# Yubo-Shankui/Bind-Your-Avatar-Implementation

Measured on AMD Instinct MI355X. Metric: denoise-steps/sec, higher is better.
Workload: dtype bf16; 1 GPU; BASELINE.json configs[1]: full transformer.forward, 49x480x720 (13x30x45 latent tokens + 226 text), 2 characters (2 ID + 2 audio), batch 1, random-init 8.6B-param architecture; layers=42, batch=1, launch=eager, parallelism=single GPU

## Files before the change

bind_your_avatar_implementation_amd/_hip.py:

```python
import ctypes
import os

from .build import LIB_PATH as _BUILT_LIB

LIB_PATH = os.environ.get("BYA_HIP_LIB") or _BUILT_LIB

_c = ctypes
_vp, _i32, _i64, _f32 = _c.c_void_p, _c.c_int32, _c.c_int64, _c.c_float


class GemmDesc(_c.Structure):
    _fields_ = [("M", _i32), ("N", _i32), ("K", _i32), ("batch", _i32),
                ("lda", _i32), ("ldw", _i32), ("ldc", _i32), ("ldres", _i32),
                ("a_batch_stride", _i64), ("c_batch_stride", _i64), ("res_batch_stride", _i64),
                ("gate_batch_stride", _i64), ("gate_split", _i32), ("act", _i32),
                ("n_split", _i32), ("c_split_stride", _i64), ("bias_rowscale", _vp), ("alpha", _f32)]


class GemmPlan(_c.Structure):
    _fields_ = [("path", _i32), ("m0", _i32), ("tail", _i32), ("split_k", _i32), ("row_chunks", _i32)]


class QkNormDesc(_c.Structure):
    _fields_ = [("qw", _vp), ("qb", _vp), ("kw", _vp), ("kb", _vp), ("cos", _vp), ("sin", _vp),
# ... 91 lines not shown

class SchedCoef(_c.Structure):
    _fields_ = [("guidance", _f32), ("sqrt_alpha", _f32), ("sqrt_beta", _f32), ("k_sample", _f32),
                ("k_denoised", _f32), ("k_noise", _f32), ("k_cur", _f32), ("k_old", _f32)]


SIGNATURES = {
    "bya_abi_version": [],
    "bya_set_option": [_i32, _i32],
    "bya_get_option": [_i32, _c.POINTER(_i32)],
    "bya_mfma_calibration": [_vp, _i64, _vp, _i32, _vp],
    "bya_gemm_bf16": [_vp, _vp, _vp, _vp, _vp, _vp, _vp, _c.POINTER(GemmDesc), _vp],
    "bya_gemm_skinny_bf16": [_vp, _vp, _vp, _vp, _vp, _c.POINTER(GemmDesc), _vp],
    "bya_gemm_qkv_norm_rope": [_vp, _vp, _vp, _vp, _c.POINTER(GemmDesc), _c.POINTER(QkNormDesc), _vp],
    "bya_gemm_bf16_plan": [_vp, _vp, _vp, _vp, _vp, _vp, _vp, _c.POINTER(GemmDesc), _c.POINTER(GemmPlan)],
    "bya_gemm_qkv_norm_rope_plan": [_vp, _vp, _vp, _vp, _c.POINTER(GemmDesc), _c.POINTER(QkNormDesc), _c.POINTER(GemmPlan)],
    "bya_gemm_qkv_norm_rope_stats": [_vp, _vp, _vp, _vp, _c.POINTER(GemmDesc), _c.POINTER(QkNormDesc), _vp, _i32, _vp],
    "bya_gemm_qkv_norm_rope_stats_plan": [_vp, _vp, _vp, _vp, _c.POINTER(GemmDesc), _c.POINTER(QkNormDesc), _vp, _i32, _c.POINTER(GemmPlan)],
    "bya_set_gemm_workspace": [_vp, _i64],
    "bya_gemm_workspace_bytes": [_c.POINTER(_i64)],
    "bya_gemm_workspace_status": [_c.POINTER(_i32), _vp],
    "bya_quantize_rows_fp8": [_vp, _vp, _vp, _i32, _i32, _i64, _i64, _vp],
    "bya_gemm_fp8": [_vp, _vp, _vp, _vp, _vp, _vp, _vp, _vp, _vp, _c.POINTER(GemmDesc), _vp],
    "bya_gemm_fp8_plan": [_vp, _vp, _vp, _vp, _vp, _vp, _vp, _vp, _vp, _c.POINTER(GemmDesc), _c.POINTER(GemmPlan)],
    "bya_gemm_fp8_qkv_norm_rope": [_vp, _vp, _vp, _vp, _vp, _vp, _c.POINTER(GemmDesc), _c.POINTER(QkNormDesc), _vp],
    "bya_gemm_fp8_qkv_norm_rope_plan": [_vp, _vp, _vp, _vp, _vp, _vp, _c.POINTER(GemmDesc), _c.POINTER(QkNormDesc),
                                        _c.POINTER(GemmPlan)],
    "bya_gemm_fp8_qkv_norm_rope_stats": [_vp, _vp, _vp, _vp, _vp, _vp, _c.POINTER(GemmDesc), _c.POINTER(QkNormDesc), _vp, _i32, _vp],
    "bya_gemm_fp8_qkv_norm_rope_stats_plan": [_vp, _vp, _vp, _vp, _vp, _vp, _c.POINTER(GemmDesc), _c.POINTER(QkNormDesc), _vp, _i32,
                                              _c.POINTER(GemmPlan)],
# ... 101 lines not shown
    "bya_p2p_push_verified": [_vp, _i32, _i64, _vp, _i32, _i32, _vp, _vp, _vp, _vp, _vp, _vp],
    "bya_p2p_exchange_verified": [_vp, _i32, _i64, _vp, _i32, _i32, _vp, _vp, _i64, _vp, _vp, _vp, _vp, _vp],
    "bya_p2p_verify": [_vp, _vp, _vp, _i32, _i32, _vp, _vp, _vp],
    "bya_p2p_poison": [_vp, _i32, _vp, _i64, _vp],
    "bya_p2p_alloc": [_i64, _i32, _c.POINTER(_vp)],
    "bya_p2p_free": [_vp],
    "bya_p2p_ipc_export": [_vp, _vp],
    "bya_p2p_ipc_import": [_vp, _c.POINTER(_vp)],
    "bya_p2p_ipc_release": [_vp],
    "bya_cfg_scheduler_step": [_vp, _i32, _i64, _vp, _vp, _vp, _vp, _vp, _i64, _c.POINTER(SchedCoef), _vp],
    "bya_cfg_scheduler_step_plan": [_vp, _i32, _i64, _vp, _vp, _i64, _c.POINTER(SchedCoef), _c.POINTER(StepPlan)],
}

OPTIONS = {"gemm_splitk": 0, "gemm_splitk_min": 1, "gemm_tile": 2, "gemm_variant": 3, "attn_streamk": 4, "fp8_kernel": 5,
           "p2p_groups": 6, "reference_forms": 7, "mx_kernel": 8}
REFERENCE_FORMS = {"rowgemm_chunked": 1, "kv_mix_generic": 2, "ln_generic": 4, "router_scores_wave": 8, "attn_narrow_store": 16}
def _named_value(var, v, table):
    if v not in table:
        raise ValueError(f"{var}={v!r}: expected one of {sorted(table)}")
    return table[v]


ENV_OPTIONS = {
    "BYA_GEMM_SPLITK": ("gemm_splitk", int),
    "BYA_GEMM_SPLITK_MIN": ("gemm_splitk_min", int),
    "BYA_GEMM_TILE": ("gemm_tile", int),
    "BYA_GEMM_VARIANT": ("gemm_variant", lambda v: {"w8": 1, "no128": 2}.get(v, 0)),
    "BYA_ATTN_STREAMK": ("attn_streamk", int),
    "BYA_FP8_KERNEL": ("fp8_kernel", lambda v: 1 if v.startswith("1") else 0),
    "BYA_P2P_GROUPS": ("p2p_groups", int),
    "BYA_MX_KERNEL": ("mx_kernel", lambda v: _named_value("BYA_MX_KERNEL", v, {"0": 0, "1": 1, "p256": 1, "2": 2, "always": 2})),
# ... 69 lines not shown
```

bind_your_avatar_implementation_amd/csrc/gemm.hip:

```cpp
#include "gemm_common.h"
#include <stdlib.h>
#include <string.h>
#include "options.h"

namespace {


template <int ROWS, int NWAVES>
__device__ __forceinline__ void stage_tile(const bf16_t* __restrict__ src, int ld, int row0, int row_max, int k0,
                                           char* lds_tile, int wave, int lane) {
    constexpr int PER_WAVE = ROWS / NWAVES;
#pragma unroll
    for (int q = 0; q < PER_WAVE / 8; ++q) {
        const int rbase = wave * PER_WAVE + q * 8;
        const int rl = rbase + (lane >> 3);
        const int chunk = (lane & 7) ^ ((rl >> 1) & 7);
        int gr = row0 + rl;
        gr = gr < row_max ? gr : row_max;
        const bf16_t* g = src + (long long)gr * ld + k0 + chunk * 8;
        __builtin_amdgcn_global_load_lds(GLOBAL_PTR(g), LDS_PTR(lds_tile + rbase * 128), 16, 0, 0);
    }
}

__device__ __forceinline__ bf16x8 lds_frag(const char* tile, int row, int chunk) {
// ... 211 lines not shown
            load_frag_b<0>(bx, cW0);
            if (t + 2 < nk) { piece(t + 2, 0); piece(t + 2, 1); }
        }
        __builtin_amdgcn_sched_barrier(0);
        mfma_quadrant<1, 0>(acc, a1, by);
        __builtin_amdgcn_sched_barrier(0);
    }
    asm volatile("s_waitcnt lgkmcnt(0)" ::: "memory");

    auto run = [&](auto act_tag) {
        epilogue_block<decltype(act_tag)::value, 4, 8, 2>(p, z, m0 + wm * 128 + fr, n0 + wn * 64 + fq * 4, acc);
    };
    dispatch_act_big(p.act, run);
}

inline bool v4_eligible(const GemmArgs& a) {
    return a.K >= 3 * BK && a.N % 8 == 0 && a.n_split % 8 == 0 && a.ldc % 8 == 0 && (!a.res || a.ldres % 8 == 0) &&
        !(((uintptr_t)a.C | (uintptr_t)a.res | (uintptr_t)a.bias | (uintptr_t)a.gate0 | (uintptr_t)a.gate1) & 15) &&
        a.c_bs % 8 == 0 && a.res_bs % 8 == 0 && a.gate_bs % 8 == 0 && a.c_split_stride % 8 == 0;
}

inline bool p128_eligible(const GemmArgs& a) { return v4_eligible(a) && a.K >= 4 * BK && a.conv_cpg_log2 < 0 && bya_opt(BYA_OPT_GEMM_VARIANT) == 0; }

inline int path256(const GemmArgs& a) {
    return v4_eligible(a) && bya_opt(BYA_OPT_GEMM_VARIANT) != 1 ? BYA_GEMM_PATH_P256 : BYA_GEMM_PATH_W8_256;
}

int launch_w8_256(const GemmArgs& a, int batch, hipStream_t s) {
    const int tiles_m = (a.M + 255) / 256, tiles_n = (a.N + 255) / 256;
    dim3 grid(tiles_m * tiles_n, 1, batch);
    const size_t lds = 2 * 512 * BK * 2;
    static std::atomic<unsigned long long> attr_done{0};
    if (bya_allow_big_lds(reinterpret_cast<const void*>(gemm256_kernel), (int)lds, attr_done) != BYA_OK) return BYA_ERR_LAUNCH;
    BYA_LAUNCH(gemm256_kernel, grid, dim3(512), lds, s, a);
    return hipGetLastError() == hipSuccess ? BYA_OK : BYA_ERR_LAUNCH;
}

// ... 2 lines not shown
    const int tiles_m = (a.M + BM - 1) / BM, tiles_n = (a.N + BN - 1) / BN;
    dim3 grid(tiles_m * tiles_n, 1, batch);
    const size_t lds = 2 * (BM + BN) * BK * 2;
    static std::atomic<unsigned long long> attr_done{0};
    if (bya_allow_big_lds(reinterpret_cast<const void*>(gemm_bf16_kernel<BM, BN, WAVES_M, WAVES_N>), (int)lds, attr_done) != BYA_OK)
        return BYA_ERR_LAUNCH;
    BYA_LAUNCH((gemm_bf16_kernel<BM, BN, WAVES_M, WAVES_N>), grid, dim3(64 * WAVES_M * WAVES_N), lds, s, a);
    return hipGetLastError() == hipSuccess ? BYA_OK : BYA_ERR_LAUNCH;
}

constexpr double REL_128S = 0.85, REL_128P = 0.80;
inline double rounds_128(int M, int N, int batch, double rel) {
    const long long t = (long long)((M + 127) / 128) * ((N + 255) / 256) * batch;
    return 0.5 * (double)((t + 255) / 256) / rel;
}
inline double rounds_256_split(int M, int N, int K, int batch) {
    const long long tiles = (long long)((M + 255) / 256) * ((N + 255) / 256) * batch, full = tiles / 256, rem = tiles % 256;
    if (rem == 0) return (double)full;
    const int R = (int)((rem + 7) / 8);
    int parts = 32 / R;
    const int by_k = (K / BK) / bya_gemm_split_min_ktiles();
    if (parts > by_k) parts = by_k;
    return (double)full + (parts > 1 ? 1.0 / parts + 0.3 : 1.0);
}
inline int hybrid_rows(int M, int N, int batch, double rel, double* cost) {
    const long long tn = (N + 255) / 256, tiles = (long long)((M + 255) / 256) * tn, full = tiles / 256;
    if (batch != 1 || full < 1 || tiles % 256 == 0) return 0;
    const int main_tm = (int)(full * 256 / tn), m0 = main_tm * 256;
    if (m0 <= 0 || m0 >= M) return 0;
    *cost = (double)(((long long)main_tm * tn + 255) / 256) + rounds_128(M - m0, N, 1, rel) + 0.05;
    return m0;
}
inline int plan_rows_qkn(int M, int N, int batch, int* m0) {
    const int forced = bya_opt(BYA_OPT_GEMM_TILE);
    if (forced >= 0) return forced == 5 || forced == 6 ? 1 : 0;
    const long long t256 = (long long)((M + 255) / 256) * ((N + 255) / 256) * batch;
    const double r256 = (double)((t256 + 255) / 256), r128 = rounds_128(M, N, batch, REL_128P);
    double best = r256, hc = 0.0;
    int plan = 0;
    if (r128 < 0.97 * best) { best = r128; plan = 1; }
    const int hm = hybrid_rows(M, N, batch, REL_128P, &hc);
    if (hm > 0 && hc < (plan == 0 ? r256 - 0.15 : 0.97 * best)) { *m0 = hm; plan = 2; }
    return plan;
}

// ... 9 lines not shown
    const double t256x128 = rounds(256, 128, 1) / 0.95;
    const double frac_rounds = (double)((M + 255) / 256) * ((N + 255) / 256) * batch / 256.0;
    const double t256 = splitk ? (frac_rounds + 0.12) * 65536.0 : rounds(256, 256, 1) / 1.00;
    (void)t256x128;
#ifdef BYA_GEMM_NO_DEEP_GRID
    const bool deep_grid = false;
#else
    const bool deep_grid = frac_rounds >= 4.0 && M >= 512 && K >= 512;
#endif
    if (((M < 1024 || K < 1024) && !deep_grid) || N < 512 || !act_on_big_tiles(act)) return 1;
    if (p128_ok) {
        const double t256s = (splitk ? rounds_256_split(M, N, K, batch) * 65536.0 : t256) / 1.2;
        const double best = t256s <= t128 ? t256s : t128, r128 = rounds_128(M, N, batch, REL_128S);
        if (r128 * 65536.0 / 1.2 < 0.97 * best) {
            double hc = 0.0;
            if (!splitk && hybrid_rows(M, N, batch, REL_128S, &hc) > 0 && hc < 0.97 * r128 && t256 / 1.2 <= t128) return 4;
            return 6;
        }
    }
    return (t256 / 1.2 <= t128) ? 4 : 1;
}

}

namespace {
constexpr int MAX_DEVICES = 64;
std::atomic<void*> g_gemm_ws[MAX_DEVICES];
inline int current_device() {
    int dev = 0;
    return hipGetDevice(&dev) == hipSuccess && dev >= 0 && dev < MAX_DEVICES ? dev : -1;
}
// ... 15 lines not shown
    if (!ws) return BYA_OK;
    unsigned word = 0;
    if (hipMemcpyAsync(&word, ws + 1023 * 4, 4, hipMemcpyDeviceToHost, stream) != hipSuccess) return BYA_ERR_LAUNCH;
    if (hipStreamSynchronize(stream) != hipSuccess) return BYA_ERR_LAUNCH;
    *timeouts = (int32_t)word;
    return BYA_OK;
}

extern "C" int bya_gemm_workspace_bytes(int64_t* bytes) {
    if (!bytes) return BYA_ERR_SHAPE;
    *bytes = (int64_t)GEMM_WS_BYTES;
    return BYA_OK;
}

namespace {
int dispatch_gemm(const GemmArgs& a, int nbatch, hipStream_t stream, bya_gemm_plan* plan);

int bf16_args(const void* A, const void* W, const void* bias, const void* C, const void* res, const void* gate0,
              const void* gate1, const bya_gemm_desc* d, GemmArgs* out) {
    if (!A || !W || !C || !d) return BYA_ERR_SHAPE;
    if (d->M <= 0 || d->N <= 0 || d->K <= 0 || d->batch <= 0) return BYA_ERR_SHAPE;
    if (d->K % BK != 0 || d->N % 4 != 0) return BYA_ERR_SHAPE;
    if (d->lda % 8 || d->ldw % 8) return BYA_ERR_ALIGN;
    if (((uintptr_t)A | (uintptr_t)W) & 15) return BYA_ERR_ALIGN;
    const int rc = gemm_epilogue_check(C, res, bias, gate0, gate1, d, d->act >= 0 && d->act <= 6);
    if (rc != BYA_OK) return rc;
    gemm_fill_args(A, W, bias, C, res, gate0, gate1, d, out);
    const int dev = current_device();
    char* const ws = dev < 0 ? nullptr : static_cast<char*>(g_gemm_ws[dev].load());
    out->ws_counters = reinterpret_cast<unsigned*>(ws);
    out->ws_slabs = ws ? reinterpret_cast<float*>(ws + GEMM_WS_COUNTER_BYTES) : nullptr;
// ... 9 lines not shown
    if (rcs != BYA_OK) return rcs;
    if (d->M <= 0 || d->N <= 0 || d->K <= 0 || d->batch <= 0 || d->K % BK != 0) return BYA_ERR_SHAPE;
    if ((d->N != 3 * n->width && d->N != 2 * n->width) || n->width % 128 != 0 || d->n_split <= 0 || d->act != 0 || d->bias_rowscale || (d->alpha != 0.0f && d->alpha != 1.0f))
        return BYA_ERR_UNSUPPORTED;
    if (d->lda % 8 || d->ldw % 8) return BYA_ERR_ALIGN;
    if (((uintptr_t)A | (uintptr_t)W | (uintptr_t)C | (uintptr_t)bias | (uintptr_t)n->qw | (uintptr_t)n->qb | (uintptr_t)n->kw |
         (uintptr_t)n->kb | (uintptr_t)n->cos | (uintptr_t)n->sin) & 15) return BYA_ERR_ALIGN;
    gemm_fill_args(A, W, bias, C, nullptr, nullptr, nullptr, d, out);
    out->ldres = 0; out->res_bs = 0; out->gate_bs = 0; out->gate_split = 0;
    qkn_fill_norm(n, out);
    if (!v4_eligible(*out) || !gemm_rows_reachable(*out, out->M)) return BYA_ERR_UNSUPPORTED;
    return qkn_stats_args(d, n, st, out);
}

int bf16_gemm(const void* A, const void* W, const void* bias, const void* C, const void* res, const void* gate0,
              const void* gate1, const bya_gemm_desc* d, hipStream_t stream, bya_gemm_plan* plan) {
    GemmArgs a;
    const int rc = bf16_args(A, W, bias, C, res, gate0, gate1, d, &a);
    if (rc != BYA_OK) return rc;
    return gemm_row_chunks(a, d->batch, 2, plan, [&](const GemmArgs& piece, int batch, long long) {
        return dispatch_gemm(piece, batch, stream, plan);
    });
}

int qkn_gemm(const void* A, const void* W, const void* bias, const void* C, const bya_gemm_desc* d, const bya_qknorm_desc* n,
             const QknStats& st, hipStream_t stream, bya_gemm_plan* plan) {
    GemmArgs a;
    const int rc0 = qkn_args(A, W, bias, C, d, n, st, &a);
    if (rc0 != BYA_OK) return rc0;
    int m0 = 0;
    const int rows = p128_eligible(a) ? plan_rows_qkn(a.M, a.N, d->batch, &m0) : 0;
    if (plan) {
        gemm_plan_whole(plan, rows == 1 ? BYA_GEMM_PATH_P128 : BYA_GEMM_PATH_P256, 1);
        if (rows == 2) { plan->m0 = m0; plan->tail = BYA_GEMM_PATH_P128; }
        return BYA_OK;
    }
// ... 4 lines not shown
        return rc != BYA_OK ? rc : bya_launch_gemm128p_qkn(&hi, 1, stream);
    }
    return bya_launch_gemm256p_qkn(&a, d->batch, stream);
}
}

extern "C" int bya_gemm_bf16(const void* A, const void* W, const void* bias, void* C, const void* res,
                             const void* gate0, const void* gate1, const bya_gemm_desc* d, hipStream_t stream) {
    return bf16_gemm(A, W, bias, C, res, gate0, gate1, d, stream, nullptr);
}

extern "C" int bya_gemm_bf16_plan(const void* A, const void* W, const void* bias, const void* C, const void* res,
                                  const void* gate0, const void* gate1, const bya_gemm_desc* d, bya_gemm_plan* plan) {
    if (!plan) return BYA_ERR_SHAPE;
    return bf16_gemm(A, W, bias, C, res, gate0, gate1, d, nullptr, plan);
}

extern "C" int bya_gemm_qkv_norm_rope(const void* A, const void* W, const void* bias, void* C, const bya_gemm_desc* d,
                                      const bya_qknorm_desc* n, hipStream_t stream) {
    return qkn_gemm(A, W, bias, C, d, n, QknStats{}, stream, nullptr);
}

extern "C" int bya_gemm_qkv_norm_rope_plan(const void* A, const void* W, const void* bias, const void* C, const bya_gemm_desc* d,
                                           const bya_qknorm_desc* n, bya_gemm_plan* p) {
    if (!p) return BYA_ERR_SHAPE;
    return qkn_gemm(A, W, bias, C, d, n, QknStats{}, nullptr, p);
}

extern "C" int bya_gemm_qkv_norm_rope_stats(const void* A, const void* W, const void* bias, void* C, const bya_gemm_desc* d,
                                            const bya_qknorm_desc* n, float* stats, int32_t stats_slots, hipStream_t stream) {
// ... 99 lines not shown
    a.gate_split = fold ? nbatch : 0;
    const int rows = fold ? nbatch * a.M : a.M, mt = (rows + 15) / 16;
    const dim3 grid((unsigned)(a.N / 16), (unsigned)(fold ? 1 : nbatch));
    switch (mt) {
        case 1: return launch_skinny_mt<1>(a, grid, stream);
        case 2: return launch_skinny_mt<2>(a, grid, stream);
        case 3: return launch_skinny_mt<3>(a, grid, stream);
        case 4: return launch_skinny_mt<4>(a, grid, stream);
        case 5: return launch_skinny_mt<5>(a, grid, stream);
        case 6: return launch_skinny_mt<6>(a, grid, stream);
        case 7: return launch_skinny_mt<7>(a, grid, stream);
        default: return launch_skinny_mt<8>(a, grid, stream);
    }
}

void plan_gemm(const GemmArgs& a, int nbatch, bya_gemm_plan* p) {
    gemm_plan_whole(p, -1, 1);
    const bool ws = a.ws_counters != nullptr;
    const int forced = bya_opt(BYA_OPT_GEMM_TILE);
    const bool splitk = ws && bya_opt(BYA_OPT_GEMM_SPLITK) != 0 && a.K / BK >= 2 * bya_gemm_split_min_ktiles() && v4_eligible(a) &&
        bya_opt(BYA_OPT_GEMM_VARIANT) != 1;
    const int tile = pick_tile(a.M, a.N, a.K, nbatch, forced, a.act, splitk, p128_eligible(a));
    if (tile >= 0 && tile <= 3) { p->path = tile; return; }
    if ((tile == 5 || tile == 6) && p128_eligible(a)) { p->path = tile; return; }
    p->path = path256(a);
    const int tn = (a.N + 255) / 256, tm = (a.M + 255) / 256;
    const long long tiles = (long long)tm * tn;
    const long long full = tiles / 256;
    if (!splitk && nbatch == 1 && full >= 1 && tiles % 256 != 0) {
        const int main_tm = (int)(full * 256 / tn);
        const int m0 = main_tm * 256;
        if (m0 > 0 && m0 < a.M) {
            const long long tail_blocks = (long long)((a.M - m0 + 127) / 128) * ((a.N + 127) / 128);
            double tail_cost = 0.9 * (double)((tail_blocks + 511) / 512);
#ifdef BYA_GEMM_NO_P128_TAIL
            const bool tail_128p = false;
#else
            const bool tail_128p = p128_eligible(a) && act_on_big_tiles(a.act) && rounds_128(a.M - m0, a.N, 1, REL_128S) + 0.05 < tail_cost;
#endif
            if (tail_128p) tail_cost = rounds_128(a.M - m0, a.N, 1, REL_128S) + 0.05;
            const double main_cost = (double)(((long long)main_tm * tn + 255) / 256);
            if (main_cost + tail_cost < (double)((tiles + 255) / 256) - 0.15) {
                p->m0 = m0;
                p->tail = tail_128p ? BYA_GEMM_PATH_P128S : BYA_GEMM_PATH_T128X128;
                return;
            }
        }
    }
    if (p->path == BYA_GEMM_PATH_P256) p->split_k = bya_gemm256p_split(&a, nbatch);
}

int launch_path(int path, const GemmArgs& a, int batch, hipStream_t stream) {
    switch (path) {
        case BYA_GEMM_PATH_T128X64: return launch<128, 64, 2, 2>(a, batch, stream);
        case BYA_GEMM_PATH_T128X128: return launch<128, 128, 2, 2>(a, batch, stream);
        case BYA_GEMM_PATH_T256X128: return launch<256, 128, 4, 2>(a, batch, stream);
        case BYA_GEMM_PATH_T256X256: return launch<256, 256, 2, 4>(a, batch, stream);
        case BYA_GEMM_PATH_P256: return bya_launch_gemm256p(&a, batch, stream);
        case BYA_GEMM_PATH_P128: return bya_launch_gemm128p(&a, batch, stream);
        case BYA_GEMM_PATH_P128S: return bya_launch_gemm128s(&a, batch, stream);
        case BYA_GEMM_PATH_W8_256: return launch_w8_256(a, batch, stream);
        default: return BYA_ERR_UNSUPPORTED;
    }
}

int dispatch_gemm(const GemmArgs& a, int nbatch, hipStream_t stream, bya_gemm_plan* plan) {
    bya_gemm_plan p;
    plan_gemm(a, nbatch, &p);
    if (plan) {
        *plan = p;
        return BYA_OK;
    }
    if (p.m0 > 0) {
        const int rc = launch_path(p.path, gemm_rows(a, 0, 0, p.m0, 2), 1, stream);
        return rc != BYA_OK ? rc : launch_path(p.tail, gemm_rows(a, 0, p.m0, a.M - p.m0, 2), 1, stream);
    }
    return launch_path(p.path, a, nbatch, stream);
}
}


extern "C" int bya_gemm_skinny_bf16(const void* A, const void* W, const void* bias, void* C, const void* res,
                                    const bya_gemm_desc* d, hipStream_t stream) {
    if (!A || !W || !C || !d) return BYA_ERR_SHAPE;
    if (d->M <= 0 || d->N <= 0 || d->K <= 0 || d->batch <= 0) return BYA_ERR_SHAPE;
    if (d->act < 0 || d->act > 6) return BYA_ERR_UNSUPPORTED;
    GemmArgs a;
    gemm_fill_args(A, W, bias, C, res, nullptr, nullptr, d, &a);
    a.gate_bs = 0; a.gate_split = 0;
    if (!skinny_eligible(a)) return BYA_ERR_UNSUPPORTED;
    return launch_skinny(a, d->batch, stream);
}
// ... 1 lines not shown
```

bind_your_avatar_implementation_amd/csrc/gemm_common.h:

```cpp
#pragma once
#include "bya_common.h"
#include "../../include/bya.h"

namespace {

struct GemmArgs {
    const bf16_t* A; const bf16_t* W; const bf16_t* bias; bf16_t* C; const bf16_t* res;
    const bf16_t* gate0; const bf16_t* gate1;
    int M, N, K;
    int lda, ldw, ldc, ldres;
    long long a_bs, c_bs, res_bs, gate_bs;
    int gate_split;
    int act;
    float leaky;
    int n_split;
    long long c_split_stride;
    const float* bias_rowscale;
    float alpha;
    float* ws_slabs;
    unsigned* ws_counters;
    int gm = 4;
    const bf16_t* qkn_w[2] = {nullptr, nullptr};
    const bf16_t* qkn_b[2] = {nullptr, nullptr};
    const float* qkn_cos = nullptr; const float* qkn_sin = nullptr;
// ... 253 lines not shown
    if (!gemm_rows_reachable(a, a.M) || ((long long)a.M - a.qkn_text_rows) * 256 >= 0x7fffffffLL) return BYA_ERR_UNSUPPORTED;
    return qkn_stats_args(d, n, s, out);
}

inline int gemm_group_m(const GemmArgs& a) { return a.K >= 8192 ? 2 : (a.N >= 8192 ? 8 : 4); }

}

int bya_launch_gemm256p(const void* args, int batch, hipStream_t stream);
int bya_launch_gemm256p_qkn(const void* args, int batch, hipStream_t stream);
int bya_gemm_split_min_ktiles();
int bya_gemm256p_split(const void* args, int batch);
int bya_launch_gemm128p(const void* args, int batch, hipStream_t stream);
int bya_launch_gemm128p_qkn(const void* args, int batch, hipStream_t stream);
int bya_launch_gemm128s(const void* args, int batch, hipStream_t stream);
```

bind_your_avatar_implementation_amd/csrc/gemm_v6.hip:

```cpp
#include "gemm_wide_epilogue.h"
#include "options.h"

#ifndef BYA_GEMM6_ABLATE
#define BYA_GEMM6_ABLATE 0
#endif

namespace {

__global__ __launch_bounds__(512, 1) void gemm128s_kernel(GemmArgs p, int tiles_m, int tiles_n, int batch) {
    extern __shared__ __attribute__((aligned(16))) char smem[];
    constexpr int BM = 128, BN = 256, TILE_A = BM * BK * 2, STAGE = (BM + BN) * BK * 2;
    static_assert(TILE_A == 16384 && STAGE == 49152, "three stages fill 144 KiB");
    const int tid = threadIdx.x, lane = tid & 63;
    const int wave = __builtin_amdgcn_readfirstlane(tid >> 6);
    const int nk = p.K / BK;

    const TileWalk<BM, BN> walk(tiles_m, tiles_n, batch, p.gm);
    int seq = 0;
    PersistentTile cur = walk.coord(seq);
    if (!cur.valid) return;
    const uint32_t lds0 = (uint32_t)(uintptr_t)LDS_PTR(smem);

    if (wave >= 4) {
        const int lw = wave - 4;
// ... 300 lines not shown
        } else {
            auto run = [&](auto act_tag) {
                epilogue_wide<decltype(act_tag)::value, 1, false, false, 4>(p, cur.z, cur.m0 + wm * 64, cur.n0 + wn * 128, fr, fq, acc, wave, lane);
            };
            dispatch_act_big(p.act, run);
        }

        if (!nxt.valid) break;
        ++seq;
        cur = nxt;
    }
#undef RA
#undef RW
}

}

int bya_launch_gemm128s(const void* args, int batch, hipStream_t s) {
    GemmArgs a = *static_cast<const GemmArgs*>(args);
#ifdef BYA_GEMM6_GM
    a.gm = BYA_GEMM6_GM;
#else
    a.gm = 2 * gemm_group_m(a);
#endif
    const int tiles_m = (a.M + 127) / 128, tiles_n = (a.N + 255) / 256;
    const size_t lds = 3 * (128 + 256) * BK * 2;
    return launch_persistent<gemm128s_kernel>(persistent_grid((long long)tiles_m * tiles_n * batch), 512, lds, s, a, tiles_m, tiles_n, batch);
}
```

bind_your_avatar_implementation_amd/csrc/misc.hip:

```cpp
#include "bya_common.h"
#include "../../include/bya.h"
#include "options.h"
#include "routing_weights.h"

namespace {

template <int MAXM>
__global__ __launch_bounds__(256) void linear_small_m_kernel(const bf16_t* __restrict__ x, const bf16_t* __restrict__ W,
                                                             const bf16_t* __restrict__ bias, bf16_t* __restrict__ out,
                                                             int M, int N, int K, int silu_in, int act_out) {
    const int lane = threadIdx.x & 63;
    const long long n = (long long)blockIdx.x * 4 + (threadIdx.x >> 6);
    if (n >= N) return;
    float acc[MAXM];
#pragma unroll
    for (int m = 0; m < MAXM; ++m) acc[m] = 0.f;
    const bf16_t* wrow = W + n * K;
    for (int k0 = lane * 8; k0 < K; k0 += 512) {
        float wv[8];
        unpack8(*reinterpret_cast<const u32x4*>(wrow + k0), wv);
#pragma unroll
        for (int m = 0; m < MAXM; ++m) {
            if (m < M) {
                float xv[8];
// ... 282 lines not shown

std::atomic<int32_t> g_bya_options[BYA_OPT_COUNT] = {
    {0},
    {0},
    {-1},
    {0},
    {1},
    {0},
    {0},
    {0},
    {0},
};

extern "C" int bya_set_option(int32_t key, int32_t value) {
    static const int32_t lo[BYA_OPT_COUNT] = {0, 0, -1, 0, 0, 0, 0, 0, 0};
    static const int32_t hi[BYA_OPT_COUNT] = {2, 1 << 20, 6, 2, 1, 1, 1024, 31, 2};
    if (key < 0 || key >= BYA_OPT_COUNT || value < lo[key] || value > hi[key]) return BYA_ERR_SHAPE;
    if (key == BYA_OPT_P2P_GROUPS && value != 0 && value < 16) return BYA_ERR_SHAPE;
    g_bya_options[key].store(value, std::memory_order_relaxed);
    return BYA_OK;
}

extern "C" int bya_get_option(int32_t key, int32_t* value) {
    if (key < 0 || key >= BYA_OPT_COUNT || !value) return BYA_ERR_SHAPE;
    *value = g_bya_options[key].load(std::memory_order_relaxed);
    return BYA_OK;
}

static int small_m_plan_of(const void* x, const void* W, const void* out, int32_t M, int32_t N, int32_t K, int32_t act_out,
                           bya_step_plan_info* p) {
    if (!x || !W || !out || M <= 0 || M > 8 || N <= 0 || K <= 0) return BYA_ERR_SHAPE;
// ... 190 lines not shown
```

bind_your_avatar_implementation_amd/ops.py:

```python
import ctypes
import os

import torch

from . import _hip
from ._hip import AttnDesc, AttnMixDesc, GemmDesc, check

ACT = {None: 0, "none": 0, "gelu_tanh": 1, "gelu_erf": 2, "relu": 3, "silu": 4, "leaky_relu": 5,
       "gelu_tanh_ieee": 6}


_PINNED_STREAM = None


def _stream():
    if _PINNED_STREAM is not None:
        return _PINNED_STREAM
    return torch.cuda.current_stream().cuda_stream


class pinned_stream:

    def __enter__(self):
        global _PINNED_STREAM
# ... 417 lines not shown
def _plan_dict(p):
    return {"path": GEMM_PATHS[p.path], "m0": p.m0, "tail": GEMM_PATHS.get(p.tail) if p.m0 > 0 else None,
            "split_k": p.split_k, "row_chunks": p.row_chunks}


def plan_key(plan):
    return plan["path"] + (f"|{plan['tail']}" if plan["tail"] else "") + ("+splitk" if plan["split_k"] else "")


def gemm_plan(a, w, out, bias=None, res=None, gate0=None, gate1=None, gate_split=0, gate_batch_stride=0, act=None,
              split=None, bias_rowscale=None, alpha=1.0):
    _, call = _gemm_call(a, w, bias, out, res, gate0, gate1, split, (gate_split, gate_batch_stride, act, bias_rowscale, alpha), True)
    if call[0] == "bya_gemm_skinny_bf16":
        return {"path": "skinny", "m0": 0, "tail": None, "split_k": 0, "row_chunks": 1}
    return _plan(call)


def _qkn_call(a, w, out, bias, split, norm, tensors, plan, stats=None):
    if tensors not in (2, 3) or w.shape[0] % tensors:
        raise ValueError("gemm_qkv_norm_rope: a [(B,) M, K], w [3 * width, K] (or [2 * width, K]: q | k alone, tensors=2), "
                         "out = the first of the split outputs")
    d = _gemm_desc(a, w, out, None, tuple(split), _NO_EPILOGUE, plan)
    n = _qkn_desc(d, tensors, *norm, plan)
    q = _plan_p if plan else _p
    return d, _with_stats(("bya_gemm_qkv_norm_rope", (q(a), q(w), q(bias), q(out), ctypes.byref(d), ctypes.byref(n))), d, n, stats, plan)


def gemm_qkv_norm_rope(a, w, out, bias, split, qw, qb, kw, kb, cos, sin, text_rows, eps=1e-6, k_scale=1.0, tensors=3, stats=None):
    d, call = _qkn_call(a, w, out, bias, split, (qw, qb, kw, kb, cos, sin, text_rows, eps, k_scale), tensors, False, stats)
    return _launch(_bf16_bucket(d), None, d, call, True)
# ... 1061 lines not shown
```

include/bya.h:

```cpp
#ifndef BYA_H
#define BYA_H

#include <stdint.h>

#ifdef __cplusplus
extern "C" {
#endif
#if defined(__GNUC__) || defined(__clang__)
#pragma GCC visibility push(default)
#endif

#ifndef __HIP_PLATFORM_AMD__
typedef struct ihipStream_t* hipStream_t;
#endif

enum { BYA_ACT_NONE = 0, BYA_ACT_GELU_TANH = 1, BYA_ACT_GELU_ERF = 2, BYA_ACT_RELU = 3, BYA_ACT_SILU = 4,
       BYA_ACT_LEAKY_RELU = 5,
       BYA_ACT_GELU_TANH_IEEE = 6  };

int bya_abi_version(void);

enum bya_option {
    BYA_OPT_GEMM_SPLITK = 0,
    BYA_OPT_GEMM_SPLITK_MIN = 1,
    BYA_OPT_GEMM_TILE = 2,
    BYA_OPT_GEMM_VARIANT = 3,
    BYA_OPT_ATTN_STREAMK = 4,
    BYA_OPT_FP8_KERNEL = 5,
    BYA_OPT_P2P_GROUPS = 6,
    BYA_OPT_REFERENCE_FORMS = 7,
    BYA_OPT_MX_KERNEL = 8,
    BYA_OPT_COUNT = 9
};
enum { BYA_REF_ROWGEMM_CHUNKED = 1,
       BYA_REF_KV_MIX_GENERIC = 2,
       BYA_REF_LN_GENERIC = 4,
       BYA_REF_ROUTER_SCORES_WAVE = 8,
       BYA_REF_ATTN_NARROW_STORE = 16   };
int bya_set_option(int32_t key, int32_t value);
int bya_get_option(int32_t key, int32_t* value);

#define BYA_CALIBRATION_OPERAND_BYTES (256LL * 256 * 16 * 16)
#define BYA_CALIBRATION_FLOP_PER_ITER (256.0 * 4 * 2.0 * 128 * 128 * 32)
int bya_mfma_calibration(const void* operands, int64_t operand_bytes, void* sink, int32_t iters, hipStream_t stream);

typedef struct bya_gemm_desc {
    int32_t M, N, K;
    int32_t batch;
    int32_t lda, ldw, ldc, ldres;
    int64_t a_batch_stride, c_batch_stride, res_batch_stride, gate_batch_stride;
    int32_t gate_split;
    int32_t act;
    int32_t n_split;
// ... 30 lines not shown
#define BYA_GEMM_PATH_T256X256 3
#define BYA_GEMM_PATH_P256 4
#define BYA_GEMM_PATH_P128 5
#define BYA_GEMM_PATH_P128S 6
#define BYA_GEMM_PATH_W8_256 7
#define BYA_GEMM_PATH_COUNT 8
typedef struct bya_gemm_plan {
    int32_t path;
    int32_t m0;
    int32_t tail;
    int32_t split_k;
    int32_t row_chunks;
} bya_gemm_plan;
int bya_gemm_bf16_plan(const void* A, const void* W, const void* bias, const void* C, const void* res,
                       const void* gate0, const void* gate1, const bya_gemm_desc* desc, bya_gemm_plan* plan);
int bya_gemm_qkv_norm_rope_plan(const void* A, const void* W, const void* bias, const void* C, const bya_gemm_desc* desc,
                                const bya_qknorm_desc* norm, bya_gemm_plan* plan);
int bya_gemm_qkv_norm_rope_stats_plan(const void* A, const void* W, const void* bias, const void* C, const bya_gemm_desc* desc,
                                      const bya_qknorm_desc* norm, const float* stats, int32_t stats_slots, bya_gemm_plan* plan);

int bya_quantize_rows_fp8(const void* x, void* q, float* scale, int32_t M, int32_t K, int64_t ldx, int64_t ldq,
                          hipStream_t stream);
int bya_gemm_fp8(const void* A8, const float* a_scale, const void* W8, const float* w_scale, const void* bias, void* C,
                 const void* res, const void* gate0, const void* gate1, const bya_gemm_desc* desc, hipStream_t stream);
int bya_gemm_fp8_plan(const void* A8, const float* a_scale, const void* W8, const float* w_scale, const void* bias,
                      const void* C, const void* res, const void* gate0, const void* gate1, const bya_gemm_desc* desc,
                      bya_gemm_plan* plan);
int bya_gemm_fp8_qkv_norm_rope(const void* A8, const float* a_scale, const void* W8, const float* w_scale, const void* bias,
                               void* C, const bya_gemm_desc* desc, const bya_qknorm_desc* norm, hipStream_t stream);
int bya_gemm_fp8_qkv_norm_rope_plan(const void* A8, const float* a_scale, const void* W8, const float* w_scale,
// ... 444 lines not shown
```

Before: 2.921 steps/s.

## Add persistent 128x128 warp-specialized GEMM for thin hybrid tails

Adds a persistent 128x128-tile bf16 GEMM kernel in which four producer waves stream A and W into a three-stage LDS ring and four consumer waves run MFMA, each covering 32 rows. The planner now uses it for the leftover row tail of hybrid 256/128 GEMMs when that tail has few tiles, so more CUs get work than with 128x256 tail tiles. The aim is to shorten the partial final wave (tail quantization) on the large transformer GEMMs. It also adds a tile_n query API and a reference-form switch to fall back to the old half-width tail, at the cost of more kernel code and planner heuristics.

```diff
diff --git a/bind_your_avatar_implementation_amd/_hip.py b/bind_your_avatar_implementation_amd/_hip.py
--- a/bind_your_avatar_implementation_amd/_hip.py
+++ b/bind_your_avatar_implementation_amd/_hip.py
@@ -129,6 +129,7 @@
     "bya_gemm_skinny_bf16": [_vp, _vp, _vp, _vp, _vp, _c.POINTER(GemmDesc), _vp],
     "bya_gemm_qkv_norm_rope": [_vp, _vp, _vp, _vp, _c.POINTER(GemmDesc), _c.POINTER(QkNormDesc), _vp],
     "bya_gemm_bf16_plan": [_vp, _vp, _vp, _vp, _vp, _vp, _vp, _c.POINTER(GemmDesc), _c.POINTER(GemmPlan)],
+    "bya_gemm_bf16_tile_n": [_vp, _vp, _vp, _vp, _vp, _vp, _vp, _c.POINTER(GemmDesc), _c.POINTER(_i32)],
     "bya_gemm_qkv_norm_rope_plan": [_vp, _vp, _vp, _vp, _c.POINTER(GemmDesc), _c.POINTER(QkNormDesc), _c.POINTER(GemmPlan)],
     "bya_gemm_qkv_norm_rope_stats": [_vp, _vp, _vp, _vp, _c.POINTER(GemmDesc), _c.POINTER(QkNormDesc), _vp, _i32, _vp],
     "bya_gemm_qkv_norm_rope_stats_plan": [_vp, _vp, _vp, _vp, _c.POINTER(GemmDesc), _c.POINTER(QkNormDesc), _vp, _i32, _c.POINTER(GemmPlan)],
@@ -260,7 +261,8 @@
 
 OPTIONS = {"gemm_splitk": 0, "gemm_splitk_min": 1, "gemm_tile": 2, "gemm_variant": 3, "attn_streamk": 4, "fp8_kernel": 5,
            "p2p_groups": 6, "reference_forms": 7, "mx_kernel": 8}
-REFERENCE_FORMS = {"rowgemm_chunked": 1, "kv_mix_generic": 2, "ln_generic": 4, "router_scores_wave": 8, "attn_narrow_store": 16}
+REFERENCE_FORMS = {"rowgemm_chunked": 1, "kv_mix_generic": 2, "ln_generic": 4, "router_scores_wave": 8, "attn_narrow_store": 16,
+                   "gemm_half_tail": 32}
 def _named_value(var, v, table):
     if v not in table:
         raise ValueError(f"{var}={v!r}: expected one of {sorted(table)}")
diff --git a/bind_your_avatar_implementation_amd/csrc/gemm.hip b/bind_your_avatar_implementation_amd/csrc/gemm.hip
--- a/bind_your_avatar_implementation_amd/csrc/gemm.hip
+++ b/bind_your_avatar_implementation_amd/csrc/gemm.hip
@@ -249,13 +249,15 @@
     dispatch_act_big(p.act, run);
 }
 
-inline bool v4_eligible(const GemmArgs& a) {
-    return a.K >= 3 * BK && a.N % 8 == 0 && a.n_split % 8 == 0 && a.ldc % 8 == 0 && (!a.res || a.ldres % 8 == 0) &&
+inline bool wide_epilogue_ok(const GemmArgs& a) {
+    return a.N % 8 == 0 && a.n_split % 8 == 0 && a.ldc % 8 == 0 && (!a.res || a.ldres % 8 == 0) &&
         !(((uintptr_t)a.C | (uintptr_t)a.res | (uintptr_t)a.bias | (uintptr_t)a.gate0 | (uintptr_t)a.gate1) & 15) &&
         a.c_bs % 8 == 0 && a.res_bs % 8 == 0 && a.gate_bs % 8 == 0 && a.c_split_stride % 8 == 0;
 }
+inline bool v4_eligible(const GemmArgs& a) { return a.K >= 3 * BK && wide_epilogue_ok(a); }
 
 inline bool p128_eligible(const GemmArgs& a) { return v4_eligible(a) && a.K >= 4 * BK && a.conv_cpg_log2 < 0 && bya_opt(BYA_OPT_GEMM_VARIANT) == 0; }
+inline bool q128_eligible(const GemmArgs& a) { return wide_epilogue_ok(a) && a.K >= 2 * BK && a.conv_cpg_log2 < 0 && bya_opt(BYA_OPT_GEMM_VARIANT) == 0; }
 
 inline int path256(const GemmArgs& a) {
     return v4_eligible(a) && bya_opt(BYA_OPT_GEMM_VARIANT) != 1 ? BYA_GEMM_PATH_P256 : BYA_GEMM_PATH_W8_256;
@@ -288,6 +290,16 @@
     const long long t = (long long)((M + 127) / 128) * ((N + 255) / 256) * batch;
     return 0.5 * (double)((t + 255) / 256) / rel;
 }
+constexpr double REL_128Q = 0.70;
+inline bool thin_tail(int rows, int N) {
+    const long long tm = (rows + 127) / 128;
+    return tm * ((N + 255) / 256) <= 128 && tm * ((N + 127) / 128) <= 256;
+}
+inline double tail_rounds(int rows, int N, double rel, bool q_ok, bool* quarter) {
+    const double half = rounds_128(rows, N, 1, rel), q = 0.25 / REL_128Q;
+    *quarter = q_ok && !bya_ref_form(BYA_REF_GEMM_HALF_TAIL) && thin_tail(rows, N) && q < half;
+    return (*quarter ? q : half) + 0.05;
+}
 inline double rounds_256_split(int M, int N, int K, int batch) {
     const long long tiles = (long long)((M + 255) / 256) * ((N + 255) / 256) * batch, full = tiles / 256, rem = tiles % 256;
     if (rem == 0) return (double)full;
@@ -297,12 +309,13 @@
     if (parts > by_k) parts = by_k;
     return (double)full + (parts > 1 ? 1.0 / parts + 0.3 : 1.0);
 }
-inline int hybrid_rows(int M, int N, int batch, double rel, double* cost) {
+inline int hybrid_rows(int M, int N, int batch, double rel, double* cost, bool q_ok = false) {
     const long long tn = (N + 255) / 256, tiles = (long long)((M + 255) / 256) * tn, full = tiles / 256;
     if (batch != 1 || full < 1 || tiles % 256 == 0) return 0;
     const int main_tm = (int)(full * 256 / tn), m0 = main_tm * 256;
     if (m0 <= 0 || m0 >= M) return 0;
-    *cost = (double)(((long long)main_tm * tn + 255) / 256) + rounds_128(M - m0, N, 1, rel) + 0.05;
+    bool quarter;
+    *cost = (double)(((long long)main_tm * tn + 255) / 256) + tail_rounds(M - m0, N, rel, q_ok, &quarter);
     return m0;
 }
 inline int plan_rows_qkn(int M, int N, int batch, int* m0) {
@@ -342,7 +355,7 @@
         const double best = t256s <= t128 ? t256s : t128, r128 = rounds_128(M, N, batch, REL_128S);
         if (r128 * 65536.0 / 1.2 < 0.97 * best) {
             double hc = 0.0;
-            if (!splitk && hybrid_rows(M, N, batch, REL_128S, &hc) > 0 && hc < 0.97 * r128 && t256 / 1.2 <= t128) return 4;
+            if (!splitk && hybrid_rows(M, N, batch, REL_128S, &hc, true) > 0 && hc < 0.97 * r128 && t256 / 1.2 <= t128) return 4;
             return 6;
         }
     }
@@ -388,7 +401,7 @@
 }
 
 namespace {
-int dispatch_gemm(const GemmArgs& a, int nbatch, hipStream_t stream, bya_gemm_plan* plan);
+int dispatch_gemm(const GemmArgs& a, int nbatch, hipStream_t stream, bya_gemm_plan* plan, int32_t* tile_n = nullptr);
 
 int bf16_args(const void* A, const void* W, const void* bias, const void* C, const void* res, const void* gate0,
               const void* gate1, const bya_gemm_desc* d, GemmArgs* out) {
@@ -428,12 +441,12 @@
 }
 
 int bf16_gemm(const void* A, const void* W, const void* bias, const void* C, const void* res, const void* gate0,
-              const void* gate1, const bya_gemm_desc* d, hipStream_t stream, bya_gemm_plan* plan) {
+              const void* gate1, const bya_gemm_desc* d, hipStream_t stream, bya_gemm_plan* plan, int32_t* tile_n = nullptr) {
     GemmArgs a;
     const int rc = bf16_args(A, W, bias, C, res, gate0, gate1, d, &a);
     if (rc != BYA_OK) return rc;
     return gemm_row_chunks(a, d->batch, 2, plan, [&](const GemmArgs& piece, int batch, long long) {
-        return dispatch_gemm(piece, batch, stream, plan);
+        return dispatch_gemm(piece, batch, stream, plan, tile_n);
     });
 }
 
@@ -468,6 +481,16 @@
                                   const void* gate0, const void* gate1, const bya_gemm_desc* d, bya_gemm_plan* plan) {
     if (!plan) return BYA_ERR_SHAPE;
     return bf16_gemm(A, W, bias, C, res, gate0, gate1, d, nullptr, plan);
+}
+
+extern "C" int bya_gemm_bf16_tile_n(const void* A, const void* W, const void* bias, const void* C, const void* res,
+                                    const void* gate0, const void* gate1, const bya_gemm_desc* d, int32_t* tile_n) {
+    if (!tile_n) return BYA_ERR_SHAPE;
+    bya_gemm_plan plan;
+    int32_t n = 0;
+    const int rc = bf16_gemm(A, W, bias, C, res, gate0, gate1, d, nullptr, &plan, &n);
+    if (rc == BYA_OK) *tile_n = n;
+    return rc;
 }
 
 extern "C" int bya_gemm_qkv_norm_rope(const void* A, const void* W, const void* bias, void* C, const bya_gemm_desc* d,
@@ -597,15 +620,17 @@
     }
 }
 
-void plan_gemm(const GemmArgs& a, int nbatch, bya_gemm_plan* p) {
+void plan_gemm(const GemmArgs& a, int nbatch, bya_gemm_plan* p, int32_t* tile_n) {
     gemm_plan_whole(p, -1, 1);
+    *tile_n = 0;
     const bool ws = a.ws_counters != nullptr;
     const int forced = bya_opt(BYA_OPT_GEMM_TILE);
     const bool splitk = ws && bya_opt(BYA_OPT_GEMM_SPLITK) != 0 && a.K / BK >= 2 * bya_gemm_split_min_ktiles() && v4_eligible(a) &&
         bya_opt(BYA_OPT_GEMM_VARIANT) != 1;
     const int tile = pick_tile(a.M, a.N, a.K, nbatch, forced, a.act, splitk, p128_eligible(a));
     if (tile >= 0 && tile <= 3) { p->path = tile; return; }
-    if ((tile == 5 || tile == 6) && p128_eligible(a)) { p->path = tile; return; }
+    if ((tile == 5 || tile == 6) && p128_eligible(a)) { p->path = tile; *tile_n = tile == 6 ? 256 : 0; return; }
+    if (tile == 7 && q128_eligible(a)) { p->path = BYA_GEMM_PATH_P128S; *tile_n = 128; return; }
     p->path = path256(a);
     const int tn = (a.N + 255) / 256, tm = (a.M + 255) / 256;
     const long long tiles = (long long)tm * tn;
@@ -621,11 +646,13 @@
 #else
             const bool tail_128p = p128_eligible(a) && act_on_big_tiles(a.act) && rounds_128(a.M - m0, a.N, 1, REL_128S) + 0.05 < tail_cost;
 #endif
-            if (tail_128p) tail_cost = rounds_128(a.M - m0, a.N, 1, REL_128S) + 0.05;
+            bool tail_128q = false;
+            if (tail_128p) tail_cost = tail_rounds(a.M - m0, a.N, REL_128S, true, &tail_128q);
             const double main_cost = (double)(((long long)main_tm * tn + 255) / 256);
             if (main_cost + tail_cost < (double)((tiles + 255) / 256) - 0.15) {
                 p->m0 = m0;
                 p->tail = tail_128p ? BYA_GEMM_PATH_P128S : BYA_GEMM_PATH_T128X128;
+                *tile_n = tail_128q ? 128 : tail_128p ? 256 : 0;
                 return;
             }
         }
@@ -633,7 +660,8 @@
     if (p->path == BYA_GEMM_PATH_P256) p->split_k = bya_gemm256p_split(&a, nbatch);
 }
 
-int launch_path(int path, const GemmArgs& a, int batch, hipStream_t stream) {
+int launch_path(int path, const GemmArgs& a, int batch, hipStream_t stream, int tile_n = 0) {
+    if (path == BYA_GEMM_PATH_P128S && tile_n == 128) return bya_launch_gemm128q(&a, batch, stream);
     switch (path) {
         case BYA_GEMM_PATH_T128X64: return launch<128, 64, 2, 2>(a, batch, stream);
         case BYA_GEMM_PATH_T128X128: return launch<128, 128, 2, 2>(a, batch, stream);
@@ -647,18 +675,20 @@
     }
 }
 
-int dispatch_gemm(const GemmArgs& a, int nbatch, hipStream_t stream, bya_gemm_plan* plan) {
+int dispatch_gemm(const GemmArgs& a, int nbatch, hipStream_t stream, bya_gemm_plan* plan, int32_t* tile_n) {
     bya_gemm_plan p;
-    plan_gemm(a, nbatch, &p);
+    int32_t tn = 0;
+    plan_gemm(a, nbatch, &p, &tn);
     if (plan) {
         *plan = p;
+        if (tile_n) *tile_n = tn;
         return BYA_OK;
     }
     if (p.m0 > 0) {
         const int rc = launch_path(p.path, gemm_rows(a, 0, 0, p.m0, 2), 1, stream);
-        return rc != BYA_OK ? rc : launch_path(p.tail, gemm_rows(a, 0, p.m0, a.M - p.m0, 2), 1, stream);
-    }
-    return launch_path(p.path, a, nbatch, stream);
+        return rc != BYA_OK ? rc : launch_path(p.tail, gemm_rows(a, 0, p.m0, a.M - p.m0, 2), 1, stream, tn);
+    }
+    return launch_path(p.path, a, nbatch, stream, tn);
 }
 }
 
diff --git a/bind_your_avatar_implementation_amd/csrc/gemm_common.h b/bind_your_avatar_implementation_amd/csrc/gemm_common.h
--- a/bind_your_avatar_implementation_amd/csrc/gemm_common.h
+++ b/bind_your_avatar_implementation_amd/csrc/gemm_common.h
@@ -291,3 +291,4 @@
 int bya_launch_gemm128p(const void* args, int batch, hipStream_t stream);
 int bya_launch_gemm128p_qkn(const void* args, int batch, hipStream_t stream);
 int bya_launch_gemm128s(const void* args, int batch, hipStream_t stream);
+int bya_launch_gemm128q(const void* args, int batch, hipStream_t stream);
diff --git a/bind_your_avatar_implementation_amd/csrc/gemm_v6.hip b/bind_your_avatar_implementation_amd/csrc/gemm_v6.hip
--- a/bind_your_avatar_implementation_amd/csrc/gemm_v6.hip
+++ b/bind_your_avatar_implementation_amd/csrc/gemm_v6.hip
@@ -338,6 +338,229 @@
 #undef RW
 }
 
+#define KEEP2(F) asm volatile("" :: "v"(F[0]), "v"(F[1]))
+__global__ __launch_bounds__(512, 1) void gemm128q_kernel(GemmArgs p, int tiles_m, int tiles_n, int batch) {
+    extern __shared__ __attribute__((aligned(16))) char smem[];
+    constexpr int BM = 128, BN = 128, TILE_A = BM * BK * 2, STAGE = (BM + BN) * BK * 2;
+    static_assert(TILE_A == 16384 && STAGE == 32768, "three stages are 96 KiB");
+    const int tid = threadIdx.x, lane = tid & 63;
+    const int wave = __builtin_amdgcn_readfirstlane(tid >> 6);
+    const int nk = p.K / BK;
+
+    const TileWalk<BM, BN> walk(tiles_m, tiles_n, batch, p.gm);
+    int seq = 0;
+    PersistentTile cur = walk.coord(seq);
+    if (!cur.valid) return;
+    const uint32_t lds0 = (uint32_t)(uintptr_t)LDS_PTR(smem);
+
+    if (wave >= 4) {
+        const int lw = wave - 4;
+        uint32_t voA[4], voW[4];
+#pragma unroll
+        for (int q = 0; q < 4; ++q) {
+            const int rl = lw * 32 + q * 8 + (lane >> 3);
+            voA[q] = stage_off(lane, rl, rl, (uint32_t)(p.lda * 2));
+            voW[q] = stage_off(lane, rl, w_slot_col(rl), (uint32_t)(p.ldw * 2));
+        }
+        uint32_t fillA = __builtin_amdgcn_readfirstlane(lds0 + lw * 32 * 128);
+        uint32_t fillW = __builtin_amdgcn_readfirstlane(lds0 + TILE_A + lw * 32 * 128);
+        int fseq = 0, fk = 0;
+        i32x4 rsA = tile_rsrc_a(p, p.A, cur), rsW = tile_rsrc_w(p, p.W, cur);
+#define DMA_A(Q, BASE, RS, SOFF) DMA_PIECE(Q, BASE, voA, RS, SOFF)
+#define DMA_W(Q, BASE, RS, SOFF) DMA_PIECE(Q, BASE, voW, RS, SOFF)
+        auto fill = [&]() {
+            const uint32_t soff = (uint32_t)(fk * (BK * 2));
+            ALL4(DMA_A, fillA, rsA, soff);
+            ALL4(DMA_W, fillW, rsW, soff);
+            const bool wrap = fillA >= lds0 + 2 * STAGE;
+            fillA = wrap ? fillA - 2 * STAGE : fillA + STAGE;
+            fillW = wrap ? fillW - 2 * STAGE : fillW + STAGE;
+            if (++fk == nk) {
+                fk = 0;
+                const PersistentTile ft = walk.coord(++fseq);
+                rsA = tile_rsrc_a(p, p.A, ft);
+                rsW = tile_rsrc_w(p, p.W, ft);
+            }
+        };
+        fill();
+        fill();
+        fill();
+        asm volatile("s_waitcnt vmcnt(16)\n\ts_barrier" ::: "memory");
+        for (;;) {
+            for (int t = 0; t < nk; ++t) {
+                asm volatile("s_waitcnt vmcnt(8)\n\ts_barrier" ::: "memory");
+                fill();
+            }
+            if (!walk.coord(++seq).valid) break;
+        }
+#undef DMA_A
+#undef DMA_W
+        asm volatile("s_waitcnt vmcnt(0)" ::: "memory");
+        return;
+    }
+
+    const int fr = lane & 15, fq = lane >> 4;
+    const int a_row = wave * 32 + fr;
+    const uint32_t bA0 = frag_addr(lds0, a_row, fq), bA1 = frag_addr(lds0, a_row, 4 + fq);
+    const uint32_t bW0 = frag_addr(lds0 + TILE_A, fr, fq);
+    const uint32_t bW1 = frag_addr(lds0 + TILE_A, fr, 4 + fq);
+    uint32_t off1 = 0u, off0 = (uint32_t)STAGE;
+    uint32_t rA1 = bA1, rW1 = bW1, rA0 = bA0 + STAGE, rW0 = bW0 + STAGE;
+
+    f32x4 acc[8][2];
+    bf16x8 fa[2][2], fw[2][8];
+    asm volatile("s_barrier" ::: "memory");
+
+#define RA(S, J) ds_read128<(J) * 2048>(fa[S][J], (S) ? rA1 : rA0)
+#define RW(S, I) ds_read128<(I) * 2048>(fw[S][I], (S) ? rW1 : rW0)
+    for (;;) {
+        const PersistentTile nxt = walk.coord(seq + 1);
+        {
+            const uint32_t tA = bA0 + off1, tW = bW0 + off1;
+            ds_read128<0 * 2048>(fa[0][0], tA); ds_read128<1 * 2048>(fa[0][1], tA);
+            ds_read128<0 * 2048>(fw[0][0], tW); ds_read128<1 * 2048>(fw[0][1], tW); ds_read128<2 * 2048>(fw[0][2], tW); ds_read128<3 * 2048>(fw[0][3], tW);
+            ds_read128<4 * 2048>(fw[0][4], tW); ds_read128<5 * 2048>(fw[0][5], tW); ds_read128<6 * 2048>(fw[0][6], tW); ds_read128<7 * 2048>(fw[0][7], tW);
+            asm volatile("s_waitcnt lgkmcnt(0)" ::: "memory");
+        }
+        auto ktile = [&](auto v_c) {
+            constexpr char V = decltype(v_c)::value;
+#define MF(S, I, J) \
+            asm volatile("v_mfma_f32_16x16x32_bf16 %0, %1, %2, %0" : "+a"(acc[I][J]) : "v"(fw[S][I]), "v"(fa[S][J]))
+#define MFZ(S, I, J) \
+            asm volatile("v_mfma_f32_16x16x32_bf16 %0, %1, %2, 0" : "=a"(acc[I][J]) : "v"(fw[S][I]), "v"(fa[S][J]))
+#define SYNC() asm volatile("s_waitcnt lgkmcnt(0)\n\ts_barrier" ::: "memory")
+#define NEXT() do { \
+                asm volatile("s_waitcnt lgkmcnt(0)" ::: "memory"); \
+                off1 = off0; \
+                off0 = off0 == (uint32_t)(2 * STAGE) ? 0u : off0 + (uint32_t)STAGE; \
+                rA1 = bA1 + off1; rW1 = bW1 + off1; rA0 = bA0 + off0; rW0 = bW0 + off0; \
+            } while (0)
+        if constexpr (V == 'A') {
+            MFZ(0, 0, 0);  RA(1, 0);
+            MFZ(0, 0, 1);  RA(1, 1);
+            MFZ(0, 1, 0);  RW(1, 0);
+            MFZ(0, 1, 1);  RW(1, 1);
+            MFZ(0, 2, 0);  RW(1, 2);
+            MFZ(0, 2, 1);  RW(1, 3);
+            MFZ(0, 3, 0);  RW(1, 4);
+            MFZ(0, 3, 1);  RW(1, 5);
+            MFZ(0, 4, 0);  RW(1, 6);
+            MFZ(0, 4, 1);  RW(1, 7);
+            MFZ(0, 5, 0);
+            MFZ(0, 5, 1);
+            MFZ(0, 6, 0);
+            MFZ(0, 6, 1);
+            MFZ(0, 7, 0);
+            MFZ(0, 7, 1);  SYNC();
+            MF(1, 0, 0);  RW(0, 0);
+            MF(1, 0, 1);  RW(0, 1);
+            MF(1, 1, 0);  RW(0, 2);
+            MF(1, 1, 1);  RW(0, 3);
+            MF(1, 2, 0);  RW(0, 4);
+            MF(1, 2, 1);  RW(0, 5);
+            MF(1, 3, 0);  RW(0, 6);
+            MF(1, 3, 1);  RW(0, 7);
+            MF(1, 4, 0);  RA(0, 0);
+            MF(1, 4, 1);  RA(0, 1);
+            MF(1, 5, 0);
+            MF(1, 5, 1);
+            MF(1, 6, 0);
+            MF(1, 6, 1);
+            MF(1, 7, 0);
+            MF(1, 7, 1);  NEXT();
+        } else if constexpr (V == 'B') {
+            MF(0, 0, 0);  RA(1, 0);
+            MF(0, 0, 1);  RA(1, 1);
+            MF(0, 1, 0);  RW(1, 0);
+            MF(0, 1, 1);  RW(1, 1);
+            MF(0, 2, 0);  RW(1, 2);
+            MF(0, 2, 1);  RW(1, 3);
+            MF(0, 3, 0);  RW(1, 4);
+            MF(0, 3, 1);  RW(1, 5);
+            MF(0, 4, 0);  RW(1, 6);
+            MF(0, 4, 1);  RW(1, 7);
+            MF(0, 5, 0);
+            MF(0, 5, 1);
+            MF(0, 6, 0);
+            MF(0, 6, 1);
+            MF(0, 7, 0);
+            MF(0, 7, 1);  SYNC();
+            MF(1, 0, 0);  RW(0, 0);
+            MF(1, 0, 1);  RW(0, 1);
+            MF(1, 1, 0);  RW(0, 2);
+            MF(1, 1, 1);  RW(0, 3);
+            MF(1, 2, 0);  RW(0, 4);
+            MF(1, 2, 1);  RW(0, 5);
+            MF(1, 3, 0);  RW(0, 6);
+            MF(1, 3, 1);  RW(0, 7);
+            MF(1, 4, 0);  RA(0, 0);
+            MF(1, 4, 1);  RA(0, 1);
+            MF(1, 5, 0);
+            MF(1, 5, 1);
+            MF(1, 6, 0);
+            MF(1, 6, 1);
+            MF(1, 7, 0);
+            MF(1, 7, 1);  NEXT();
+        } else if constexpr (V == 'L') {
+            MF(0, 0, 0);  RA(1, 0);
+            MF(0, 0, 1);  RA(1, 1);
+            MF(0, 1, 0);  RW(1, 0);
+            MF(0, 1, 1);  RW(1, 1);
+            MF(0, 2, 0);  RW(1, 2);
+            MF(0, 2, 1);  RW(1, 3);
+            MF(0, 3, 0);  RW(1, 4);
+            MF(0, 3, 1);  RW(1, 5);
+            MF(0, 4, 0);  RW(1, 6);
+            MF(0, 4, 1);  RW(1, 7);
+            MF(0, 5, 0);
+            MF(0, 5, 1);
+            MF(0, 6, 0);
+            MF(0, 6, 1);
+            MF(0, 7, 0);
+            MF(0, 7, 1);  SYNC();
+            MF(1, 0, 0);
+            MF(1, 0, 1);
+            MF(1, 1, 0);
+            MF(1, 1, 1);
+            MF(1, 2, 0);
+            MF(1, 2, 1);
+            MF(1, 3, 0);
+            MF(1, 3, 1);
+            MF(1, 4, 0);
+            MF(1, 4, 1);
+            MF(1, 5, 0);
+            MF(1, 5, 1);
+            MF(1, 6, 0);
+            MF(1, 6, 1);
+            MF(1, 7, 0);
+            MF(1, 7, 1);  NEXT();
+        }
+            KEEP2(fa[0]); KEEP8(fw[0]); KEEP2(fa[1]); KEEP8(fw[1]);
+#undef MF
+#undef MFZ
+#undef SYNC
+#undef NEXT
+        };
+        ktile(IntTag<'A'>{});
+        for (int t = 1; t + 1 < nk; ++t) ktile(IntTag<'B'>{});
+        ktile(IntTag<'L'>{});
+        asm volatile("s_nop 15\n\ts_nop 15" ::: "memory");
+
+        {
+            auto run = [&](auto act_tag) {
+                epilogue_wide<decltype(act_tag)::value, 1, false, false, 2>(p, cur.z, cur.m0 + wave * 32, cur.n0, fr, fq, acc, wave, lane);
+            };
+            dispatch_act_big(p.act, run);
+        }
+
+        if (!nxt.valid) break;
+        ++seq;
+        cur = nxt;
+    }
+#undef RA
+#undef RW
+}
+
 }
 
 int bya_launch_gemm128s(const void* args, int batch, hipStream_t s) {
@@ -351,3 +574,11 @@
     const size_t lds = 3 * (128 + 256) * BK * 2;
     return launch_persistent<gemm128s_kernel>(persistent_grid((long long)tiles_m * tiles_n * batch), 512, lds, s, a, tiles_m, tiles_n, batch);
 }
+
+int bya_launch_gemm128q(const void* args, int batch, hipStream_t s) {
+    GemmArgs a = *static_cast<const GemmArgs*>(args);
+    a.gm = 2 * gemm_group_m(a);
+    const int tiles_m = (a.M + 127) / 128, tiles_n = (a.N + 127) / 128;
+    const size_t lds = 3 * (128 + 128) * BK * 2;
+    return launch_persistent<gemm128q_kernel>(persistent_grid((long long)tiles_m * tiles_n * batch), 512, lds, s, a, tiles_m, tiles_n, batch);
+}
diff --git a/bind_your_avatar_implementation_amd/csrc/misc.hip b/bind_your_avatar_implementation_amd/csrc/misc.hip
--- a/bind_your_avatar_implementation_amd/csrc/misc.hip
+++ b/bind_your_avatar_implementation_amd/csrc/misc.hip
@@ -320,7 +320,7 @@
 
 extern "C" int bya_set_option(int32_t key, int32_t value) {
     static const int32_t lo[BYA_OPT_COUNT] = {0, 0, -1, 0, 0, 0, 0, 0, 0};
-    static const int32_t hi[BYA_OPT_COUNT] = {2, 1 << 20, 6, 2, 1, 1, 1024, 31, 2};
+    static const int32_t hi[BYA_OPT_COUNT] = {2, 1 << 20, 7, 2, 1, 1, 1024, 63, 2};
     if (key < 0 || key >= BYA_OPT_COUNT || value < lo[key] || value > hi[key]) return BYA_ERR_SHAPE;
     if (key == BYA_OPT_P2P_GROUPS && value != 0 && value < 16) return BYA_ERR_SHAPE;
     g_bya_options[key].store(value, std::memory_order_relaxed);
diff --git a/bind_your_avatar_implementation_amd/ops.py b/bind_your_avatar_implementation_amd/ops.py
--- a/bind_your_avatar_implementation_amd/ops.py
+++ b/bind_your_avatar_implementation_amd/ops.py
@@ -455,6 +455,16 @@
     if call[0] == "bya_gemm_skinny_bf16":
         return {"path": "skinny", "m0": 0, "tail": None, "split_k": 0, "row_chunks": 1}
     return _plan(call)
+
+
+def gemm_tile_n(a, w, out, bias=None, res=None, gate0=None, gate1=None, gate_split=0, gate_batch_stride=0, act=None,
+                split=None, bias_rowscale=None, alpha=1.0):
+    _, call = _gemm_call(a, w, bias, out, res, gate0, gate1, split, (gate_split, gate_batch_stride, act, bias_rowscale, alpha), True)
+    if call[0] == "bya_gemm_skinny_bf16":
+        return 0
+    n = ctypes.c_int32(-1)
+    check(getattr(_hip.load(), "bya_gemm_bf16_tile_n")(*call[1], ctypes.byref(n)), "bya_gemm_bf16_tile_n")
+    return n.value
 
 
 def _qkn_call(a, w, out, bias, split, norm, tensors, plan, stats=None):
diff --git a/include/bya.h b/include/bya.h
--- a/include/bya.h
+++ b/include/bya.h
@@ -36,7 +36,8 @@
        BYA_REF_KV_MIX_GENERIC = 2,
        BYA_REF_LN_GENERIC = 4,
        BYA_REF_ROUTER_SCORES_WAVE = 8,
-       BYA_REF_ATTN_NARROW_STORE = 16   };
+       BYA_REF_ATTN_NARROW_STORE = 16,
+       BYA_REF_GEMM_HALF_TAIL = 32      };
 int bya_set_option(int32_t key, int32_t value);
 int bya_get_option(int32_t key, int32_t* value);
 
@@ -97,6 +98,8 @@
 } bya_gemm_plan;
 int bya_gemm_bf16_plan(const void* A, const void* W, const void* bias, const void* C, const void* res,
                        const void* gate0, const void* gate1, const bya_gemm_desc* desc, bya_gemm_plan* plan);
+int bya_gemm_bf16_tile_n(const void* A, const void* W, const void* bias, const void* C, const void* res,
+                         const void* gate0, const void* gate1, const bya_gemm_desc* desc, int32_t* tile_n);
 int bya_gemm_qkv_norm_rope_plan(const void* A, const void* W, const void* bias, const void* C, const bya_gemm_desc* desc,
                                 const bya_qknorm_desc* norm, bya_gemm_plan* plan);
 int bya_gemm_qkv_norm_rope_stats_plan(const void* A, const void* W, const void* bias, const void* C, const bya_gemm_desc* desc,
```

Measured after the change: 2.921 steps/s. Within noise of the previous version (-0.0%).
